# eudald-seeslab/mmsbm

Measured on AMD Instinct MI355X. Metric: EM iterations/sec (1M ratings, K=L=20), higher is better.
Workload: dtype f64; 1 GPU; C3: 1000000 synthetic ratings, 99997 users x 20000 items, R=5, K=20, L=20, one restart per GPU (sampling=1), uniform generator seed 0, model seed 0; launch=eager, pairs=99993, pair_stage=vector ALUs (pair_block_kernel)

## Files before the change

### mmsbm_amd/csrc/context.hpp

```cpp
#pragma once

namespace {

#define DISPATCH_GV(code, CALL)                                   \
  switch (code) {                                                 \
    case 0: CALL(4, 4); break;                                    \
    case 1: CALL(8, 4); break;                                    \
    case 2: CALL(16, 4); break;                                   \
    case 3: CALL(32, 4); break;                                   \
    case 4: CALL(64, 4); break;                                   \
    case 5: CALL(64, 8); break;                                   \
    default: CALL(64, 16); break;                                 \
  }

}

namespace mmsbm_hip_impl {

template <class T>
struct DevBuf {
  T *ptr = nullptr;
  size_t count = 0;
  DevBuf() = default;
  DevBuf(const DevBuf &) = delete;
// ... 153 lines not shown
}

inline void sort_unique_groups(std::vector<int32_t> &off, std::vector<int32_t> &val) {
  int32_t w = 0;
  for (size_t g = 0; g + 1 < off.size(); ++g) {
    const int32_t a = off[g], b = off[g + 1];
    std::sort(val.begin() + a, val.begin() + b);
    off[g] = w;
    for (int32_t e = a; e < b; ++e)
      if (e == a || val[e] != val[e - 1]) val[w++] = val[e];
  }
  off.back() = w;
  val.resize(static_cast<size_t>(w));
}

enum TimedCall { T_RECOMMEND = 0, T_FOLD_IN, T_POSITIONS, T_TOP_PAIRS, T_AUDIENCE, T_SIMILAR, T_OVERLAP, T_HELDOUT, T_EXPLAIN, T_DIVERSE, T_COUNT };

enum KernelId { K_SEG = 0, K_DENSE, K_ETAP, K_MATVEC_A, K_FUSED_PAIRS, K_FUSED_TAIL, K_COUNT };
const char *const kKernelNames[K_COUNT] = {"seg_pass_kernel", "pair_block_kernel(T+S)", "eta_p_kernel",
                                           "pair_block_kernel(A)", "pairs_fused_kernel", "tail_fused_kernel"};


}


struct mmsbm_hip_ctx {
  int device = 0;
  hipStream_t stream = nullptr;
  hipStream_t copy_stream = nullptr;
  hipStream_t xfer = nullptr;
  bool swapped = false;
  int64_t n_obs = 0;
  int ext_users = 0, ext_items = 0, ext_k = 0, ext_l = 0;
  int n_users = 0, n_items = 0, n_ratings = 0, k = 0, l = 0, kp = 0, lp = 0;
  int n_pairs = 0, n_chunks = 0;
  int code_k = 0, code_l = 0;
#ifdef MMSBM_ABLATE
  int ablate = 0;
#endif
  PairPlan pp;
  DevBuf<int32_t> grid_item;
  DevBuf<mmsbm::Chunk> grid_chunks;
  int grid_n_chunks = 0;
  DevBuf<double> btab;
  bool predict_fast = true;
  int seg_batch = 4;
  bool fused = false;
  bool fused_forced = false;
  bool fs_pairs = false, fs_users = false;
  DevBuf<mmsbm::FusedUnit> fp_units, fu_units;
  DevBuf<mmsbm::WorkItem> fp_items, fu_items;
  DevBuf<mmsbm::FusedSplit> fp_splits, fu_splits;
  int fp_max_parts = 0, fu_max_parts = 0, fu_blocks = 0;
  std::vector<char> a_ok;
  int nt_out = 7;
  int ranges_pairs = 1, ranges_users = 1;
  int n_cus = 256;
  bool gpu_layout = false;
  mmsbm::Layout lay;
  DevBuf<int32_t> pair_off, pair_user, pair_item, user_off, user_pair, item_off, item_pairs,
      item_deg, mv_chunk_off, orig_u, orig_i, orig_r;
  DevBuf<int32_t> item_grid;
  DevBuf<mmsbm::Chunk> mv_chunks;
  DevBuf<mmsbm::Chunk> lik_units;
  DevBuf<mmsbm::Chunk> a_chunks;
  int n_a_chunks = 0, a_units = 0;
  int n_lik_units = 0;
  DevBuf<mmsbm::WorkItem> pair_items, user_items;
  DevBuf<mmsbm::SplitSeg> pair_splits, user_splits;
  int n_slots = 1, sel = 0;
  int base_slot = 0, launch_slots = 1;
  SlotBuf pair_parts, user_parts;
  SlotBuf theta[2], eta[2], p[2], pt[2], atab[2], ctab, ttab, partial, npr;
  DevBuf<double> lik_part;
  DevBuf<double> lg_theta, lg_eta, lg_p;
  int lik_mode = 2;
  int lik_g = 0;
  PinBuf pin;
  std::unique_ptr<mmsbm_hip_impl::PredictSession> ps;
  std::unique_ptr<mmsbm_hip_impl::RecSession> rc;
  std::unique_ptr<mmsbm_hip_impl::SimSession> sm;
  std::unique_ptr<mmsbm_hip_impl::OvlSession> ov;
  std::unique_ptr<mmsbm_hip_impl::HoldSession> ho;
  std::unique_ptr<mmsbm_hip_impl::ExpSession> ex;
  float last_ms[T_COUNT] = {};
  int top_groups = 0;
  int64_t aud_rows = 0;
  int64_t aud_entries = 0;
  int64_t exp_rows = 0;
  int64_t div_rows = 0;
  DevBuf<double> snap_theta;
  SlotBuf snap_eta, snap_p;
  std::vector<char> snap_have;
  int cur = 0;
  std::vector<char> have;
  bool graph_mode = false;
  hipGraphExec_t graph_exec[2] = {nullptr, nullptr};
  bool profiling = false;
  std::vector<std::pair<int, std::pair<hipEvent_t, hipEvent_t>>> prof_events;

  void drop_graphs() {
    for (auto &g : graph_exec) {
      if (g) (void)hipGraphExecDestroy(g);
      g = nullptr;
    }
  }
// ... 65 lines not shown
```

### mmsbm_amd/csrc/launch.hpp

```cpp
#pragma once

namespace mmsbm_hip_impl {

void stage_seg(mmsbm_hip_ctx *c, bool commit, bool with_pairs, bool with_users, hipStream_t st);
void stage_dense_valu(mmsbm_hip_ctx *c);
void stage_dense_mfma(mmsbm_hip_ctx *c);
void stage_matvec_a_valu(mmsbm_hip_ctx *c, int slot, int a_slot, bool grid);
void stage_matvec_a_mfma(mmsbm_hip_ctx *c, int slot, int a_slot, bool grid);
int mfma_a_blocks_per_cu(const mmsbm_hip_ctx *c);
void stage_eta_p(mmsbm_hip_ctx *c, bool commit);
void stage_fused_pairs(mmsbm_hip_ctx *c);
void stage_fused_tail(mmsbm_hip_ctx *c, bool commit);
int likelihood_enqueue(mmsbm_hip_ctx *c);
void init_rows_launch(mmsbm_hip_ctx *c, const uint64_t pcg64_state[4]);
void omegas_launch(mmsbm_hip_ctx *c, double *dev_out, int64_t n_elems);
void prod_dist_launch(mmsbm_hip_ctx *c, const int32_t *du, const int32_t *di, double *dout, int64_t n_pairs);
int rows_launch(mmsbm_hip_ctx *c, int mode, const int32_t *pu, const int32_t *pi, const int32_t *preal,
                const double *weights, double *dist, double *block_out, int64_t n_rows, int first);
int score_rows_launch(mmsbm_hip_ctx *c, bool finish);
int score_stats_count();

void require_free_mem(size_t bytes, const std::string &what);
void recommend_begin(mmsbm_hip_ctx *c, const double *weights, int exclude_train);
void recommend_add(mmsbm_hip_ctx *c);
void recommend_query(mmsbm_hip_ctx *c, int64_t n_users, const int32_t *users, int n, int32_t *items, double *scores,
                     int32_t *counts);
void recommend_query_theta(mmsbm_hip_ctx *c, int64_t n_users, const double *theta, const int64_t *seen_offsets,
                           const int32_t *seen_items, int n, int32_t *items, double *scores, int32_t *counts);
void recommend_positions(mmsbm_hip_ctx *c, int64_t n_users, const int32_t *users, const int64_t *offsets,
                         const int32_t *items, int32_t *positions, int32_t *candidates);
void recommend_add_items(mmsbm_hip_ctx *c, int32_t n_new, const double *eta, const int64_t *seen_offsets,
                         const int32_t *seen_users);
void recommend_top_pairs(mmsbm_hip_ctx *c, int64_t n_users, const int32_t *users, int m, int32_t *out_users,
                         int32_t *out_items, double *out_scores, int32_t *count);
void recommend_query_items(mmsbm_hip_ctx *c, int64_t n_items, const int32_t *items, int n, int32_t *users,
                           double *scores, int32_t *counts);
void recommend_audience(mmsbm_hip_ctx *c, int64_t n_items, const int32_t *items, double min_score, int64_t capacity,
                        int64_t *offsets, int32_t *users, double *scores);
void recommend_query_within(mmsbm_hip_ctx *c, int64_t n_users, const int32_t *users, const int32_t *cand, int n_cand,
                            const int64_t *excl_offsets, const int32_t *excl_items, int n, int32_t *items,
                            double *scores, int32_t *counts);
void recommend_query_theta_within(mmsbm_hip_ctx *c, int64_t n_users, const double *theta, const int64_t *seen_offsets,
                                  const int32_t *seen_items, const int32_t *cand, int n_cand, int n, int32_t *items,
                                  double *scores, int32_t *counts);
void recommend_rank(mmsbm_hip_ctx *c, int64_t n_users, const int32_t *users, const int64_t *offsets,
                    const int32_t *cand, int n, int32_t *items, double *scores, int32_t *counts);
void similar_begin(mmsbm_hip_ctx *c, int side);
void similar_add(mmsbm_hip_ctx *c);
void similar_query(mmsbm_hip_ctx *c, int64_t n_rows, const int32_t *ids, int n, int32_t *out_ids, double *distance,
                   int32_t *counts);
void similar_pairs(mmsbm_hip_ctx *c, int64_t n_pairs, const int32_t *a, const int32_t *b, double *distance);
void recommend_diverse(mmsbm_hip_ctx *c, int64_t n_users, const int32_t *users, const int32_t *cand, int n_cand,
                       const int64_t *excl_offsets, const int32_t *excl_items, int n, int pool, double trade_off,
                       int32_t *items, double *scores, double *distances, int32_t *counts);
void overlap_begin(mmsbm_hip_ctx *c, int side);
void overlap_add(mmsbm_hip_ctx *c);
void overlap_query(mmsbm_hip_ctx *c, double *out);

void fold_in(mmsbm_hip_ctx *c, bool items_side, int64_t n_rows, const int32_t *user, const int32_t *item,
             const int32_t *rating, int32_t n_new, int32_t n_iters, double tol, const double *x0, double *x,
             int32_t *iters);

void heldout_begin(mmsbm_hip_ctx *c, int64_t n_rows, const int32_t *user, const int32_t *item, const int32_t *rating);
void heldout_eval(mmsbm_hip_ctx *c, int first, int n_slots, bool add, double *loglik);
void heldout_mean(mmsbm_hip_ctx *c, double *mean_p, double *loglik);
// ... 101 lines not shown
```

### mmsbm_amd/csrc/mmsbm_hip.hip

```cpp

#include "prelude.hpp"
#include "layout_gpu.hpp"
#include "pcg64.hpp"

#include <unistd.h>

#include <map>
#include <mutex>

namespace {

thread_local std::string g_last_error;

template <class F>
int guarded(F &&f) {
  try {
    f();
    return MMSBM_OK;
  } catch (const ApiError &e) {
    g_last_error = e.what();
    return e.code;
  } catch (const std::invalid_argument &e) {
    g_last_error = e.what();
    return MMSBM_E_INVALID;
// ... 81 lines not shown
}

}

namespace {

inline int balanced_run_units(const std::vector<int32_t> &rating_off, int slots, int lo, int hi) {
  int best = hi;
  double best_cost = 1e300;
  const bool align = mmsbm::chunk_align_on();
  const int n_ratings = static_cast<int>(rating_off.size()) - 1;
  for (int u = hi; u >= lo; --u) {
    long long wgs = 0;
    for (int r = 0; r < n_ratings; ++r)
      wgs += mmsbm::padded_chunk_count(rating_off[static_cast<size_t>(r) + 1] - rating_off[static_cast<size_t>(r)],
                                       u * kUnitPairs, n_ratings, align);
    const double cost = static_cast<double>((wgs + slots - 1) / std::max(slots, 1)) * (u + 0.6);
    if (cost < best_cost * 0.97) { best_cost = cost; best = u; }
  }
  return best;
}

void build_a_runs(mmsbm_hip_ctx *c, int units) {
  c->n_a_chunks = 0;
  c->a_chunks.release();
  if (!c->pp.mfma || c->n_pairs <= 0) return;
  const int now = c->pp.chunk_pairs / kUnitPairs, most = kMfmaChunkPairs / kUnitPairs;
  int a_units = units > 0 ? std::min(units, most)
                          : balanced_run_units(c->lay.rating_off, mfma_a_blocks_per_cu(c) * c->n_cus, std::max(2, now / 2),
                                               std::min(2 * now, most));
  c->a_units = a_units;
  if (a_units == now) return;
  mmsbm::Layout tmp;
  tmp.n_ratings = c->lay.n_ratings; tmp.rating_off = c->lay.rating_off;
  mmsbm::build_mv_chunks(tmp, a_units * kUnitPairs);
  c->a_chunks.upload(tmp.mv_chunks, c->stream);
  HIP_CHECK(hipStreamSynchronize(c->stream));
  c->n_a_chunks = static_cast<int>(tmp.mv_chunks.size());
}

bool fused_shape_ok(const mmsbm_hip_ctx *c) {
  return c->code_k <= 1 && c->code_l <= 1 && c->n_chunks > 0 && c->pp.fused_shape_ok();
}
bool fused_possible(const mmsbm_hip_ctx *c) {
  return fused_shape_ok(c) && (c->lay.pair_work.splits.empty() || c->fs_pairs) &&
         (c->lay.user_work.splits.empty() || c->fs_users);
}

void mark_a(mmsbm_hip_ctx *c, bool ok) {
  for (int s = c->base_slot; s < c->base_slot + c->launch_slots; ++s) c->a_ok[static_cast<size_t>(s)] = ok ? 1 : 0;
}

constexpr long long kFusedWorkMax = 14000000, kFusedWorkMaxSplit = 18000000, kFusedRatingsMax = 1500000;
bool use_fused(const mmsbm_hip_ctx *c) {
  const bool cut = !c->lay.pair_work.splits.empty() || !c->lay.user_work.splits.empty();
  return c->fused && fused_possible(c) &&
         (c->fused_forced || c->n_obs * c->launch_slots * (c->kp + c->lp) <= (cut ? kFusedWorkMaxSplit : kFusedWorkMax));
}

void launch_iteration(mmsbm_hip_ctx *c, bool commit) {
  if (use_fused(c)) {
    stage_fused_pairs(c);
    stage_fused_tail(c, commit);
    if (commit) c->cur ^= 1;
    mark_a(c, !commit);
    return;
  }
  ensure_a(c);
  stage_seg(c, commit, true, true, c->stream);
  stage_dense(c);
  stage_eta_p(c, commit);
  if (commit) {
    stage_matvec_a(c, c->cur ^ 1, c->cur ^ 1);
    c->cur ^= 1;
    mark_a(c, true);
  }
}

void run_iterations(mmsbm_hip_ctx *c, int n) {
  if (c->graph_mode && !c->profiling) {
    while (n >= 2) {
      const int slot = c->cur;
      if (!c->graph_exec[slot]) {
        if (!use_fused(c)) ensure_a(c);
        hipGraph_t graph = nullptr;
        HIP_CHECK(hipStreamBeginCapture(c->stream, hipStreamCaptureModeThreadLocal));
        try {
          launch_iteration(c, true);
          launch_iteration(c, true);
        } catch (...) {
          (void)hipStreamEndCapture(c->stream, &graph);
          if (graph) (void)hipGraphDestroy(graph);
          c->cur = slot;
          throw;
        }
        HIP_CHECK(hipStreamEndCapture(c->stream, &graph));
        hipError_t e = hipGraphInstantiate(&c->graph_exec[slot], graph, nullptr, nullptr, 0);
        (void)hipGraphDestroy(graph);
        if (e != hipSuccess)
          throw ApiError(MMSBM_E_HIP, std::string("hipGraphInstantiate: ") + hipGetErrorString(e));
      }
      HIP_CHECK(hipGraphLaunch(c->graph_exec[slot], c->stream));
      mark_a(c, !use_fused(c));
      n -= 2;
    }
  }
  for (; n > 0; --n) launch_iteration(c, true);
}

void require_params(const mmsbm_hip_ctx *c) {
  if (!c) throw std::invalid_argument("null context");
  if (!c->have[c->sel]) throw std::invalid_argument("set_params has not been called");
}
void require_all_params(const mmsbm_hip_ctx *c) {
  if (!c) throw std::invalid_argument("null context");
  for (int s = 0; s < c->n_slots; ++s)
    if (!c->have[s])
      throw std::invalid_argument(c->n_slots == 1 ? std::string("set_params has not been called")
                                                  : "set_params has not been called for slot " +
                                                        std::to_string(s));
}

void alloc_state(mmsbm_hip_ctx *c, int slots) {
// ... 434 lines not shown
                                            std::to_string(MMSBM_HIP_RECOMMEND_MAX_N) + " " + noun + " a query returns at most");
}

struct Option {
  const char *name;
  double (*get)(const mmsbm_hip_ctx *);
  void (*set)(mmsbm_hip_ctx *, double);
};
using Ctx = mmsbm_hip_ctx;
void set_audience(int64_t &field, const char *name, double v) {
  if (v < 0 || v > 2147483647.0 || v != std::floor(v)) throw std::invalid_argument(std::string(name) + ": 0 .. 2^31 - 1");
  field = static_cast<int64_t>(v);
}
const Option kOptions[] = {
    {"graph", [](const Ctx *c) -> double { return c->graph_mode; }, [](Ctx *c, double v) { c->graph_mode = v != 0.0; }},
    {"quad", [](const Ctx *c) -> double { return c->pp.quad_a; }, [](Ctx *c, double v) { c->pp.set_quad(v != 0.0); }},
    {"mfma", [](const Ctx *c) -> double { return c->pp.mfma ? 1.0 : (c->pp.mfma_big ? 2.0 : 0.0); },
     [](Ctx *c, double v) { c->pp.set_mfma(v); }},
    {"predict_fast", [](const Ctx *c) -> double { return c->predict_fast; }, [](Ctx *c, double v) { c->predict_fast = v != 0.0; }},
    {"fused", [](const Ctx *c) -> double { return c->fused; },
     [](Ctx *c, double v) {
       if (v != 0.0 && !fused_possible(c)) throw std::invalid_argument("fused: not available for this shape / data");
       c->fused = c->fused_forced = v != 0.0;
     }},
    {"nt_out", [](const Ctx *c) -> double { return nt_on(c); },
     [](Ctx *c, double v) {
       if (v < 0 || v > 15) throw std::invalid_argument("nt_out: 0 .. 15");
       c->nt_out = static_cast<int>(v);
     }},
    {"recommend_ms", [](const Ctx *c) -> double { return c->last_ms[T_RECOMMEND]; }, nullptr},
    {"fold_in_ms", [](const Ctx *c) -> double { return c->last_ms[T_FOLD_IN]; }, nullptr},
    {"position_ms", [](const Ctx *c) -> double { return c->last_ms[T_POSITIONS]; }, nullptr},
    {"similar_ms", [](const Ctx *c) -> double { return c->last_ms[T_SIMILAR]; }, nullptr},
    {"top_pairs_ms", [](const Ctx *c) -> double { return c->last_ms[T_TOP_PAIRS]; }, nullptr},
    {"overlap_ms", [](const Ctx *c) -> double { return c->last_ms[T_OVERLAP]; }, nullptr},
    {"heldout_ms", [](const Ctx *c) -> double { return c->last_ms[T_HELDOUT]; }, nullptr},
    {"audience_ms", [](const Ctx *c) -> double { return c->last_ms[T_AUDIENCE]; }, nullptr},
    {"explain_ms", [](const Ctx *c) -> double { return c->last_ms[T_EXPLAIN]; }, nullptr},
    {"diverse_ms", [](const Ctx *c) -> double { return c->last_ms[T_DIVERSE]; }, nullptr},
    {"top_pairs_groups", [](const Ctx *c) -> double { return c->top_groups; },
     [](Ctx *c, double v) {
       if (v < 0 || v > 4096 || v != std::floor(v)) throw std::invalid_argument("top_pairs_groups: 0 .. 4096");
       c->top_groups = static_cast<int>(v);
     }},
    {"audience_rows", [](const Ctx *c) -> double { return static_cast<double>(c->aud_rows); },
     [](Ctx *c, double v) { set_audience(c->aud_rows, "audience_rows", v); }},
    {"audience_entries", [](const Ctx *c) -> double { return static_cast<double>(c->aud_entries); },
     [](Ctx *c, double v) { set_audience(c->aud_entries, "audience_entries", v); }},
    {"explain_rows", [](const Ctx *c) -> double { return static_cast<double>(c->exp_rows); },
     [](Ctx *c, double v) { set_audience(c->exp_rows, "explain_rows", v); }},
    {"diverse_rows", [](const Ctx *c) -> double { return static_cast<double>(c->div_rows); },
     [](Ctx *c, double v) { set_audience(c->div_rows, "diverse_rows", v); }},
    {"launches", [](const Ctx *c) -> double { return use_fused(c) ? 2 : 4; }, nullptr},
    {"wide", [](const Ctx *c) -> double { return c->pp.wide; }, nullptr},
    {"lik_fast", [](const Ctx *c) -> double { return c->lik_mode; },
     [](Ctx *c, double v) {
       if (v != 0.0 && v != 1.0 && v != 2.0) throw std::invalid_argument("lik_fast: 0, 1 or 2");
       c->lik_mode = static_cast<int>(v);
     }},
    {"lik_g", [](const Ctx *c) -> double { return c->lik_g; },
     [](Ctx *c, double v) {
       const int g = static_cast<int>(v);
       if (g != 0 && g != 1 && g != 2 && g != 4 && g != 8) throw std::invalid_argument("lik_g: 0, 1, 2, 4 or 8");
       c->lik_g = g;
     }},
    {"ranges_pairs", [](const Ctx *c) -> double { return c->ranges_pairs; }, nullptr},
    {"ranges_users", [](const Ctx *c) -> double { return c->ranges_users; }, nullptr},
    {"chunk_pairs", [](const Ctx *c) -> double { return c->pp.chunk_pairs; }, nullptr},
    {"n_chunks", [](const Ctx *c) -> double { return c->n_chunks; }, nullptr},
    {"a_units", [](const Ctx *c) -> double { return c->a_units; },
     [](Ctx *c, double v) {
       if (v < 0 || v > kMfmaChunkPairs / kUnitPairs) throw std::invalid_argument("a_units: 0 .. 16");
       use_device(c);
       HIP_CHECK(hipStreamSynchronize(c->stream));
       build_a_runs(c, static_cast<int>(v));
     }},
    {"a_chunks", [](const Ctx *c) -> double { return c->n_a_chunks; }, nullptr},
    {"items_pairs", [](const Ctx *c) -> double { return static_cast<double>(c->lay.pair_work.items.size()); }, nullptr},
    {"items_users", [](const Ctx *c) -> double { return static_cast<double>(c->lay.user_work.items.size()); }, nullptr},
    {"splits_pairs", [](const Ctx *c) -> double { return static_cast<double>(c->lay.pair_work.splits.size()); }, nullptr},
    {"splits_users", [](const Ctx *c) -> double { return static_cast<double>(c->lay.user_work.splits.size()); }, nullptr},
    {"fused_split", [](const Ctx *c) -> double { return (c->fs_pairs ? 1 : 0) + (c->fs_users ? 2 : 0); }, nullptr},
    {"item_grid", [](const Ctx *c) -> double { return c->item_grid.count ? 1 : 0; }, nullptr},
    {"gpu_layout", [](const Ctx *c) -> double { return c->gpu_layout ? 1 : 0; }, nullptr},
};
const Option *find_option(const std::string &name) {
  for (const Option &o : kOptions)
    if (name == o.name) return &o;
  return nullptr;
}
void set_option(mmsbm_hip_ctx *ctx, const std::string &name, double value) {
  const Option *o = find_option(name);
  if (!o || !o->set) throw std::invalid_argument("unknown option: " + name);
  o->set(ctx, value);
  ctx->drop_graphs();
}
}


extern "C" {

int mmsbm_hip_abi_version(void) { return MMSBM_HIP_ABI_VERSION; }

#ifndef MMSBM_BUILD_ID
#define MMSBM_BUILD_ID "unknown"
#endif
// ... 1057 lines not shown
                            const int32_t *rating, int32_t n_new, int32_t n_iters, double tol,
                            const double *eta0, double *eta, int32_t *iters) {
  return fold_entry(ctx, true, n_rows, user, item, rating, n_new, n_iters, tol, eta0, eta, iters);
}

int mmsbm_hip_time_iterations(mmsbm_hip_ctx *ctx, int n_iters, float *elapsed_ms) {
  return guarded([&] {
    require_all_params(ctx);
    if (!elapsed_ms || n_iters < 0) throw std::invalid_argument("bad argument");
    use_device(ctx);
    EventPair ev;
    ev.start(ctx->stream);
    run_iterations(ctx, n_iters);
    ev.stop(ctx->stream);
    ev.wait();
    *elapsed_ms = ev.ms();
  });
}

int mmsbm_hip_kernel_count(void) { return K_COUNT; }

const char *mmsbm_hip_kernel_name(int index) {
  return (index >= 0 && index < K_COUNT) ? kKernelNames[index] : "";
}

int mmsbm_hip_profile_iterations(mmsbm_hip_ctx *ctx, int n_iters, float *mean_us,
                                 int *launches_per_iter) {
  return guarded([&] {
    require_all_params(ctx);
    if (!mean_us || n_iters <= 0) throw std::invalid_argument("bad argument");
    use_device(ctx);
    HIP_CHECK(hipStreamSynchronize(ctx->stream));
    ctx->profiling = true;
    try {
      for (int it = 0; it < n_iters; ++it) launch_iteration(ctx, true);
      HIP_CHECK(hipStreamSynchronize(ctx->stream));
    } catch (...) {
      ctx->profiling = false;
      throw;
    }
    ctx->profiling = false;
    collect_profile(ctx, mean_us, launches_per_iter, n_iters);
  });
}

int mmsbm_hip_kernel_bytes(const mmsbm_hip_ctx *ctx, int index, int64_t *bytes_read,
                           int64_t *bytes_written) {
  return guarded([&] {
    if (!ctx || !bytes_read || !bytes_written) throw std::invalid_argument("null argument");
    const int64_t N = ctx->n_obs, U = ctx->n_users, I = ctx->n_items, R = ctx->n_ratings;
    const int64_t K = ctx->k, L = ctx->l, Q = ctx->n_pairs;
    const int64_t C = static_cast<int64_t>(ctx->lay.mv_chunks.size());
    int64_t rd = 0, wr = 0;
    switch (index) {
      case K_SEG:
        rd = 2 * N * (4 + 8 * K) + (U + Q) * (8 * K + 4);
        wr = (U + Q) * 8 * K;
        break;
      case K_DENSE:
        rd = Q * (8 * K + 8 * L + 4) + C * 8 * K * L;
        wr = Q * 8 * L + C * 8 * K * L;
        break;
      case K_ETAP:
        rd = C * 8 * K * L + R * 8 * K * L + Q * (8 * L + 4) + I * (8 * L + 8);
        wr = 3 * R * 8 * K * L + I * 8 * L;
        break;
      case K_MATVEC_A: rd = Q * (8 * L + 4) + C * 8 * K * L; wr = Q * 8 * K; break;
      case K_FUSED_PAIRS:
        rd = Q * (8 * L + 4 + 4) + N * (4 + 8 * K) + 2 * C * 8 * K * L;
        wr = Q * (8 * K + 8 * L) + C * 8 * K * L;
        break;
      case K_FUSED_TAIL:
        rd = N * (4 + 8 * K) + U * (8 * K + 4) + C * 8 * K * L + R * 8 * K * L + Q * (8 * L + 4) + I * (8 * L + 8);
        wr = U * 8 * K + 3 * R * 8 * K * L + I * 8 * L;
        break;
      default: throw std::invalid_argument("kernel index out of range");
    }
    *bytes_read = rd * ctx->n_slots;
    *bytes_written = wr * ctx->n_slots;
  });
}

int mmsbm_hip_time_stage(mmsbm_hip_ctx *ctx, int stage, int reps, float *mean_us) {
  return guarded([&] {
    require_all_params(ctx);
#ifdef MMSBM_ABLATE
    ctx->ablate = stage >> 8;
    stage &= 0xff;
    struct Reset { mmsbm_hip_ctx *c; ~Reset() { c->ablate = 0; } } reset{ctx};
#else
    if (stage >> 8)
      throw ApiError(MMSBM_E_UNSUPPORTED, "time_stage: phase ablation (stage bits 8+) needs the diagnostic build (-DMMSBM_ABLATE, csrc/unity.hip)");
#endif
    if (!mean_us || reps <= 0 || stage < 0 || stage >= K_COUNT)
      throw std::invalid_argument("bad argument");
    if ((stage == K_FUSED_PAIRS || stage == K_FUSED_TAIL) && !fused_possible(ctx))
      throw std::invalid_argument("time_stage: the two-launch kernels do not apply to this shape / data");
    use_device(ctx);
    ensure_a(ctx);
    auto one = [&] {
      switch (stage) {
        case K_SEG: stage_seg(ctx, true, true, true, ctx->stream); break;
        case K_DENSE: stage_dense(ctx); break;
        case K_ETAP: stage_eta_p(ctx, true); break;
        case K_FUSED_PAIRS: stage_fused_pairs(ctx); break;
        case K_FUSED_TAIL: stage_fused_tail(ctx, true); break;
        default: stage_matvec_a(ctx, ctx->cur, ctx->cur ^ 1); break;
      }
    };
    for (int w = 0; w < 3; ++w) one();
    EventPair ev;
    ev.start(ctx->stream);
    for (int r = 0; r < reps; ++r) one();
    ev.stop(ctx->stream);
    ev.wait();
    *mean_us = ev.ms() * 1000.f / reps;
  });
}

int mmsbm_hip_set_option(mmsbm_hip_ctx *ctx, const char *name, double value) {
  return guarded([&] {
    if (!ctx || !name) throw std::invalid_argument("null argument");
    set_option(ctx, name, value);
  });
}

int mmsbm_hip_get_option(const mmsbm_hip_ctx *ctx, const char *name, double *value) {
  return guarded([&] {
    if (!ctx || !name || !value) throw std::invalid_argument("null argument");
    const Option *o = find_option(name);
    if (!o) throw std::invalid_argument(std::string("unknown option: ") + name);
    *value = o->get(ctx);
  });
}

int mmsbm_hip_set_graph_mode(mmsbm_hip_ctx *ctx, int enabled) {
  return guarded([&] {
    if (!ctx) throw std::invalid_argument("null context");
    set_option(ctx, "graph", enabled != 0);
  });
}

#ifdef MMSBM_STAMPS
int mmsbm_hip_debug_stamps(unsigned long long *out, int n_words) {
  return guarded([&] {
    HIP_CHECK(hipDeviceSynchronize());
    HIP_CHECK(hipMemcpyFromSymbol(out, HIP_SYMBOL(g_stamps), sizeof(unsigned long long) * n_words));
  });
}
#endif

struct mmsbm_hip_layout {
  mmsbm::Layout lay;
};

// ... 113 lines not shown
```

### mmsbm_amd/csrc/pair_plan.hpp

```cpp
#pragma once

namespace mmsbm_hip_impl {

#define MMSBM_PAIR_BLOCK_T_LIST(X)                                                                                     \
  X(1, false, 256, 2, false) X(1, false, 512, 2, false)                                                                \
  X(1, false, 256, 4, true) X(1, false, 512, 4, true) X(1, true, 256, 4, true) X(1, true, 512, 4, true)                \
  X(2, false, 256, 4, true) X(2, false, 512, 4, true) X(2, true, 256, 4, true) X(2, true, 512, 4, true)                \
  X(4, false, 512, 4, true)
#define MMSBM_PAIR_BLOCK_A_LIST(X)                                                                                     \
  X(1, false, 256, 4, false) X(1, false, 512, 4, false)                                                                \
  X(1, false, 256, 4, true) X(1, false, 512, 4, true) X(1, true, 256, 4, true) X(1, true, 512, 4, true)

constexpr int pair_block_key(int nacc, bool tlds, int nt, int kt, bool direct) {
  return nacc | (kt << 4) | (tlds ? 1 << 8 : 0) | (direct ? 1 << 9 : 0) | (nt << 10);
}
#define MMSBM_PB_LISTED(N, TL, NT, KT, D) case pair_block_key(N, TL, NT, KT, D):
inline bool pair_block_t_listed(int key) {
  switch (key) { MMSBM_PAIR_BLOCK_T_LIST(MMSBM_PB_LISTED) return true; default: return false; }
}
inline bool pair_block_a_listed(int key) {
  switch (key) { MMSBM_PAIR_BLOCK_A_LIST(MMSBM_PB_LISTED) return true; default: return false; }
}
#undef MMSBM_PB_LISTED

enum class PairForm { Wide, Block, Quad, Mfma, MfmaBig };

struct PairPlan {
  int kp = 0, lp = 0;
  int threads_t = kBlock, threads_a = kBlock;
  int kt = 4;
  int spb = kBlock, nacc = 1, nsub = 1;
  bool tl_t = false, tl_a = false;
  size_t lds_t = 0, lds_a = 0;
  bool direct_out = false;
  bool wide = false;
  bool mfma = false;
  bool mfma_big = false;
  bool quad_a = false;
  size_t lds_mt = 0, lds_ma = 0, lds_qa = 0;
  int chunk_pairs = mmsbm::kMvChunkPairs;

  bool big_tile() const { return tile_beyond_scalar_cache(kp, lp); }
  bool mfma_possible() const {
    return !wide && kp <= kMfmaMaxDim && lp <= kMfmaMaxDim && lds_mt <= kLdsMax && lds_ma <= kLdsMax;
  }
  bool quad_possible() const {
    return !wide && big_tile() && tl_a && threads_a == kPairBlockMax && lds_qa <= kLdsMax - 2048 && lp <= kQuadMaxL;
  }
  bool on_mfma() const { return mfma || mfma_big; }
  bool fused_shape_ok() const {
    return threads_t == kBlock && threads_a == kBlock && !tl_t && !tl_a && nacc == 1 && kt == 2 && spb * nsub <= kBlock &&
           !wide && !mfma && !mfma_big && !direct_out && chunk_pairs == mmsbm::kMvChunkPairs &&
           pairs_fused_lds(kp, lp) <= kLdsBudget;
  }

  PairForm form_t() const {
    return mfma_big ? PairForm::MfmaBig : mfma ? PairForm::Mfma : wide ? PairForm::Wide : PairForm::Block;
  }
  PairForm form_a() const { return (!on_mfma() && !wide && quad_a) ? PairForm::Quad : form_t(); }
  int key_t() const { return pair_block_key(nacc, tl_t, threads_t, kt, direct_out); }
  int key_a() const { return pair_block_key(1, tl_a, threads_a, 4, direct_out); }
  int quad_nl() const {
    const int nl = (lp + 3) / 4;
    return nl <= 8 ? 8 : nl <= 10 ? 10 : nl <= 12 ? 12 : nl <= 13 ? 13 : 14;
  }

  void set_mfma(double value) {
    mfma = value == 1.0 && mfma_possible();
    mfma_big = value != 0.0 && !mfma && chunk_pairs <= kMfmaChunkPairs;
  }
  void set_quad(bool on) { quad_a = on && quad_possible(); }
};

inline PairPlan plan_pair_shape(int kp, int lp, bool force_wide) {
  PairPlan p;
  p.kp = kp; p.lp = lp;
  auto threads_for = [](int nch) { return nch <= 6 ? kBlock : kPairBlockMax; };
  p.threads_t = threads_for(lp / 4);
  p.threads_a = threads_for(kp / 4);
  const int nthr = p.threads_t;
  p.kt = ((kp / 2) * (lp / 4) <= kBlock / 2) ? 2 : 4;
  const int nslot = (kp / p.kt) * (lp / 4);
  if (nslot <= nthr / 2) {
    p.spb = nslot; p.nacc = 1;
    const int room = (kp * (kUnitPairs + 1) + kUnitPairs * lp) / (nslot * 4 * p.kt);
    p.nsub = std::max(1, std::min(std::min(nthr / nslot, 8), 1 + room));
  } else {
    p.spb = nthr;
    int n = 1;
    while (n * nthr < nslot) n *= 2;
    p.nacc = n;
  }
  p.tl_t = tile_in_lds(kp, lp);
  p.tl_a = tile_in_lds(lp, kp);
  p.lds_t = pair_block_lds(kp, lp, p.tl_t);
  p.lds_a = pair_block_lds(lp, kp, p.tl_a);
  if (p.lds_t > kLdsMax) { p.tl_t = false; p.lds_t = pair_block_lds(kp, lp, false); }
  if (p.lds_a > kLdsMax) { p.tl_a = false; p.lds_a = pair_block_lds(lp, kp, false); }
  p.wide = p.lds_t > kLdsMax || p.lds_a > kLdsMax || p.nacc > 4 || force_wide;
  return p;
}

inline PairPlan plan_pair_forms(PairPlan p, int n_pairs, int n_cus, bool no_mfma, int mfma_chunk) {
  const bool big_tile = p.big_tile();
  p.lds_mt = pair_mfma_lds(p.kp, p.lp, true);
  p.lds_ma = pair_mfma_lds(p.lp, p.kp, false);
// ... 14 lines not shown
```

### mmsbm_amd/csrc/tu_fused.hip

```cpp
#include "prelude.hpp"
#include "seg_pass.hpp"
#include "pair_block.hpp"
#include "eta_p.hpp"
#include "fused_small.hpp"

namespace mmsbm_hip_impl {

void stage_fused_pairs(mmsbm_hip_ctx *c) {
  LaunchScope ls(c, K_FUSED_PAIRS, true);
  const int s = c->base_slot, cur = c->cur;
  FusedPairArgs fa{};
  fa.pt_tiles = c->pt[cur].at(s); fa.p_tiles = c->p[cur].at(s); fa.eta = c->eta[cur].at(s);
  fa.theta = theta_tab(c, cur); fa.a_out = a_tab(c, cur);
  fa.pair_off = c->pair_off.ptr; fa.pair_user = c->pair_user.ptr; fa.pair_item = c->pair_item.ptr;
  fa.chunks = c->mv_chunks.ptr; fa.t_out = c->ttab.at(s); fa.partial = c->partial.at(s);
  fa.kp = c->kp; fa.lp = c->lp; fa.spb = c->pp.spb; fa.nsub = c->pp.nsub; fa.nt = nt_on(c) & 1;
  fa.bs_tiles = c->p[0].stride; fa.bs_eta = c->eta[0].stride; fa.bs_t = c->ttab.stride; fa.bs_partial = c->partial.stride;
  const bool split = c->fs_pairs && !c->lay.pair_work.splits.empty();
  fa.units = split ? c->fp_units.ptr : nullptr; fa.items = split ? c->fp_items.ptr : nullptr;
  fa.splits = split ? c->fp_splits.ptr : nullptr;
  const size_t lds = pairs_fused_lds(c->kp, c->lp, split ? c->fp_max_parts : 0);
  const dim3 grid = slot_grid(c, c->n_chunks);
#define PF(G, S)                                                                  \
  do {                                                                            \
    allow_big_lds(pairs_fused_kernel<G, 4, S>, lds);                              \
    LAUNCH_IN(ls, (pairs_fused_kernel<G, 4, S>), grid, kBlock, lds, c->stream, fa); \
  } while (0)
  if (c->code_k == 0) { if (split) PF(4, true); else PF(4, false); }
  else { if (split) PF(8, true); else PF(8, false); }
#undef PF
  ls.done();
}
void stage_fused_tail(mmsbm_hip_ctx *c, bool commit) {
  LaunchScope ls(c, K_FUSED_TAIL, true);
  const SegArgs su = seg_users_args(c, commit, c->n_users);
  const EtaPArgs a = eta_p_args(c, commit, kRedCols);
  const int per_u = kBlock / group_lanes(c->code_k), per_i = kBlock / group_lanes(c->code_l);
  const bool split = c->fs_users && !c->lay.user_work.splits.empty();
  const int bu = split ? c->fu_blocks : (su.nseg + per_u - 1) / per_u, nb_i = (c->n_items + per_i - 1) / per_i;
  const dim3 grid = slot_grid(c, bu + a.nb_p + nb_i);
  const FusedUserArgs fu{split ? c->fu_units.ptr : nullptr, split ? c->fu_items.ptr : nullptr, split ? c->fu_splits.ptr : nullptr};
  const size_t lds = split ? static_cast<size_t>(c->fu_max_parts) * c->kp * sizeof(double) : 0;
  const bool deep = static_cast<long long>(grid.x) * grid.y <= c->n_cus;
#define TAIL(G, V, GL, VL)                                                                                        \
  do {                                                                                                            \
    if (split) {                                                                                                  \
      allow_big_lds(tail_fused_kernel<G, V, GL, VL, 16, true>, lds);                                              \
      LAUNCH_IN(ls, (tail_fused_kernel<G, V, GL, VL, 16, true>), grid, kBlock, lds, c->stream, su, a, bu, c->kp, fu); \
    } else if (deep) LAUNCH_IN(ls, (tail_fused_kernel<G, V, GL, VL, 32, false>), grid, kBlock, 0, c->stream, su, a, bu, c->kp, fu); \
    else LAUNCH_IN(ls, (tail_fused_kernel<G, V, GL, VL, 16, false>), grid, kBlock, 0, c->stream, su, a, bu, c->kp, fu);      \
  } while (0)
  switch (c->code_k * 2 + c->code_l) {
    case 0: TAIL(4, 4, 4, 4); break;
    case 1: TAIL(4, 4, 8, 4); break;
    case 2: TAIL(8, 4, 4, 4); break;
    default: TAIL(8, 4, 8, 4); break;
  }
#undef TAIL
  ls.done();
}

}
```

Measured before the change: 10650 it/s.

## Merge pair segment pass and dense tile stage into one kernel for large shapes

Adds a pass_dense kernel that, per chunk of pairs, computes the pair-side theta gather and normalisation, builds the T output and the partial K×L tile sums in LDS, and runs the user segment pass as extra blocks of the same launch. It replaces the separate stage_seg and stage_dense launches on commit iterations when the shape qualifies (code_k==1, no splits, work at or above a threshold). The aim is to cut one launch and avoid writing and re-reading the pair-side intermediate through global memory. The cost is heavier LDS use and lower occupancy per block. The two-launch fused path and the original path are left as they were.

Result: faster. 11840 it/s, median of 6 (+11.2%).

```diff
diff --git a/mmsbm_amd/csrc/context.hpp b/mmsbm_amd/csrc/context.hpp
--- a/mmsbm_amd/csrc/context.hpp
+++ b/mmsbm_amd/csrc/context.hpp
@@ -229,6 +229,7 @@
   DevBuf<mmsbm::WorkItem> fp_items, fu_items;
   DevBuf<mmsbm::FusedSplit> fp_splits, fu_splits;
   int fp_max_parts = 0, fu_max_parts = 0, fu_blocks = 0;
+  int pass_dense = -1;
   std::vector<char> a_ok;
   int nt_out = 7;
   int ranges_pairs = 1, ranges_users = 1;
diff --git a/mmsbm_amd/csrc/launch.hpp b/mmsbm_amd/csrc/launch.hpp
--- a/mmsbm_amd/csrc/launch.hpp
+++ b/mmsbm_amd/csrc/launch.hpp
@@ -11,6 +11,7 @@
 void stage_eta_p(mmsbm_hip_ctx *c, bool commit);
 void stage_fused_pairs(mmsbm_hip_ctx *c);
 void stage_fused_tail(mmsbm_hip_ctx *c, bool commit);
+void stage_pass_dense(mmsbm_hip_ctx *c);
 int likelihood_enqueue(mmsbm_hip_ctx *c);
 void init_rows_launch(mmsbm_hip_ctx *c, const uint64_t pcg64_state[4]);
 void omegas_launch(mmsbm_hip_ctx *c, double *dev_out, int64_t n_elems);
diff --git a/mmsbm_amd/csrc/mmsbm_hip.hip b/mmsbm_amd/csrc/mmsbm_hip.hip
--- a/mmsbm_amd/csrc/mmsbm_hip.hip
+++ b/mmsbm_amd/csrc/mmsbm_hip.hip
@@ -157,10 +157,24 @@
 }
 
 constexpr long long kFusedWorkMax = 14000000, kFusedWorkMaxSplit = 18000000, kFusedRatingsMax = 1500000;
+
+bool pass_dense_possible(const mmsbm_hip_ctx *c) {
+  return c->launch_slots == 1 && c->code_k == 1 && c->code_l <= 1 && c->n_chunks > 0 && c->pp.pass_dense_shape_ok() &&
+         c->lay.pair_work.items.empty() && c->lay.user_work.items.empty() && c->lay.pair_work.splits.empty() &&
+         c->lay.user_work.splits.empty();
+}
+constexpr long long kPassDenseWorkMin = 20000000;
+static_assert(kPassDenseWorkMin > kFusedWorkMaxSplit, "no shape changes from two launches to three");
+
 bool use_fused(const mmsbm_hip_ctx *c) {
   const bool cut = !c->lay.pair_work.splits.empty() || !c->lay.user_work.splits.empty();
+  if (c->pass_dense == 1 && !c->fused_forced && pass_dense_possible(c)) return false;
   return c->fused && fused_possible(c) &&
          (c->fused_forced || c->n_obs * c->launch_slots * (c->kp + c->lp) <= (cut ? kFusedWorkMaxSplit : kFusedWorkMax));
+}
+bool use_pass_dense(const mmsbm_hip_ctx *c) {
+  if (c->pass_dense == 0 || use_fused(c) || !pass_dense_possible(c)) return false;
+  return c->pass_dense == 1 || c->n_obs * (c->kp + c->lp) >= kPassDenseWorkMin;
 }
 
 void launch_iteration(mmsbm_hip_ctx *c, bool commit) {
@@ -172,8 +186,12 @@
     return;
   }
   ensure_a(c);
-  stage_seg(c, commit, true, true, c->stream);
-  stage_dense(c);
+  if (commit && use_pass_dense(c)) {
+    stage_pass_dense(c);
+  } else {
+    stage_seg(c, commit, true, true, c->stream);
+    stage_dense(c);
+  }
   stage_eta_p(c, commit);
   if (commit) {
     stage_matvec_a(c, c->cur ^ 1, c->cur ^ 1);
@@ -714,6 +732,11 @@
     {"diverse_rows", [](const Ctx *c) -> double { return static_cast<double>(c->div_rows); },
      [](Ctx *c, double v) { set_audience(c->div_rows, "diverse_rows", v); }},
     {"launches", [](const Ctx *c) -> double { return use_fused(c) ? 2 : 4; }, nullptr},
+    {"pass_dense", [](const Ctx *c) -> double { return use_pass_dense(c) ? 1 : 0; },
+     [](Ctx *c, double v) {
+       if (v != -1.0 && v != 0.0 && v != 1.0) throw std::invalid_argument("pass_dense: -1, 0 or 1");
+       c->pass_dense = static_cast<int>(v);
+     }},
     {"wide", [](const Ctx *c) -> double { return c->pp.wide; }, nullptr},
     {"lik_fast", [](const Ctx *c) -> double { return c->lik_mode; },
      [](Ctx *c, double v) {
@@ -1877,12 +1900,18 @@
     const int64_t K = ctx->k, L = ctx->l, Q = ctx->n_pairs;
     const int64_t C = static_cast<int64_t>(ctx->lay.mv_chunks.size());
     int64_t rd = 0, wr = 0;
+    const bool merged = use_pass_dense(ctx);
     switch (index) {
       case K_SEG:
         rd = 2 * N * (4 + 8 * K) + (U + Q) * (8 * K + 4);
         wr = (U + Q) * 8 * K;
+        if (merged) {
+          rd += Q * (8 * L + 4) + C * 8 * K * L;
+          wr += Q * (8 * L - 8 * K) + C * 8 * K * L;
+        }
         break;
       case K_DENSE:
+        if (merged) break;
         rd = Q * (8 * K + 8 * L + 4) + C * 8 * K * L;
         wr = Q * 8 * L + C * 8 * K * L;
         break;
@@ -1923,9 +1952,17 @@
       throw std::invalid_argument("time_stage: the two-launch kernels do not apply to this shape / data");
     use_device(ctx);
     ensure_a(ctx);
+    const bool merged = use_pass_dense(ctx);
+    if (merged && stage == K_DENSE) {
+      *mean_us = 0.f;
+      return;
+    }
     auto one = [&] {
       switch (stage) {
-        case K_SEG: stage_seg(ctx, true, true, true, ctx->stream); break;
+        case K_SEG:
+          if (merged) stage_pass_dense(ctx);
+          else stage_seg(ctx, true, true, true, ctx->stream);
+          break;
         case K_DENSE: stage_dense(ctx); break;
         case K_ETAP: stage_eta_p(ctx, true); break;
         case K_FUSED_PAIRS: stage_fused_pairs(ctx); break;
diff --git a/mmsbm_amd/csrc/pair_plan.hpp b/mmsbm_amd/csrc/pair_plan.hpp
--- a/mmsbm_amd/csrc/pair_plan.hpp
+++ b/mmsbm_amd/csrc/pair_plan.hpp
@@ -52,6 +52,10 @@
     return threads_t == kBlock && threads_a == kBlock && !tl_t && !tl_a && nacc == 1 && kt == 2 && spb * nsub <= kBlock &&
            !wide && !mfma && !mfma_big && !direct_out && chunk_pairs == mmsbm::kMvChunkPairs &&
            pairs_fused_lds(kp, lp) <= kLdsBudget;
+  }
+  bool pass_dense_shape_ok() const {
+    return form_t() == PairForm::Block && threads_t == kBlock && !tl_t && nacc == 1 && kt == 2 && spb * nsub <= kBlock &&
+           !direct_out && chunk_pairs == mmsbm::kMvChunkPairs && kUnitPairs * lp <= 3 * 2 * kBlock && lds_t <= kLdsBudget;
   }
 
   PairForm form_t() const {
diff --git a/mmsbm_amd/csrc/pass_dense.hpp b/mmsbm_amd/csrc/pass_dense.hpp
--- /dev/null
+++ b/mmsbm_amd/csrc/pass_dense.hpp
@@ -0,0 +1,217 @@
+#pragma once
+
+namespace {
+
+struct PassDenseArgs {
+  RowTab a_fixed;
+  RowTab theta;
+  const int32_t *pair_off, *pair_user, *pair_item;
+  const mmsbm::Chunk *chunks;
+  const double *p_tiles;
+  const double *eta;
+  double *t_out;
+  double *partial;
+  int kp, lp, spb, nsub;
+  int nt;
+  int n_units;
+};
+
+template <int G, int VEC>
+__device__ __forceinline__ void pass_dense_unit(const PassDenseArgs &pa, int unit) {
+  constexpr int CS = kUnitPairs + 1, KT = 2, TV = KT * 4, B = 4;
+  constexpr int NGRP = kBlock / G, ROUNDS = kUnitPairs / NGRP;
+  constexpr int CH = (G < 16) ? 2 * G : G;
+  constexpr int NE = 3;
+  const int kp = pa.kp, lp = pa.lp;
+  extern __shared__ double lds[];
+  double *cst = lds;
+  double *es = cst + static_cast<size_t>(kp) * CS;
+  double *tout = es;
+  const mmsbm::Chunk ch = pa.chunks[unit];
+  const int tid = threadIdx.x, wave = tid >> 6, lane = tid & 63;
+  const int q0 = ch.q_begin, np = ch.q_end - ch.q_begin;
+  const int grp = tid / G, gl = tid % G;
+  typedef const double __attribute__((address_space(4))) * const_tile_ptr;
+  const const_tile_ptr gtile = (const_tile_ptr)(reinterpret_cast<uintptr_t>(
+      pa.p_tiles + static_cast<size_t>(ch.rating) * kp * lp));
+
+  int beg[ROUNDS], end[ROUNDS], ids[NE];
+  const int tot = np * lp;
+#pragma unroll
+  for (int r = 0; r < ROUNDS; ++r) {
+    const int p = grp + r * NGRP;
+    beg[r] = p < np ? pa.pair_off[q0 + p] : 0;
+    end[r] = p < np ? pa.pair_off[q0 + p + 1] : 0;
+  }
+#pragma unroll
+  for (int j = 0; j < NE; ++j) {
+    const int t = min(tid * 2 + j * kBlock * 2, max(tot - 2, 0));
+    ids[j] = tot > 0 ? pa.pair_item[q0 + t / lp] : 0;
+  }
+  const auto eta_row = [&](int j) {
+    const int t = min(tid * 2 + j * kBlock * 2, max(tot - 2, 0));
+    return *reinterpret_cast<const double2 *>(pa.eta + static_cast<size_t>(ids[j]) * lp + t % lp);
+  };
+  const double2 ev0 = eta_row(0), ev1 = eta_row(1), ev2 = eta_row(2);
+  int m0, m1;
+  {
+    const int cnt = min(CH, end[0] - beg[0]);
+    m0 = cnt > 0 ? pa.pair_user[beg[0] + min(gl, cnt - 1)] : 0;
+    m1 = (CH > G && cnt > 0) ? pa.pair_user[beg[0] + min(G + gl, cnt - 1)] : 0;
+  }
+  __builtin_amdgcn_sched_barrier(0);
+  if (tid * 2 < tot) *reinterpret_cast<double2 *>(es + tid * 2) = ev0;
+  if (tid * 2 + kBlock * 2 < tot) *reinterpret_cast<double2 *>(es + tid * 2 + kBlock * 2) = ev1;
+  if (tid * 2 + kBlock * 4 < tot) *reinterpret_cast<double2 *>(es + tid * 2 + kBlock * 4) = ev2;
+
+  const bool act = gl * VEC < kp;
+  const int lane_off = act ? gl * VEC : 0;
+  const bool g_main = lane_off < pa.theta.mw;
+  const double *gbase = g_main ? pa.theta.main + lane_off : pa.theta.tail + (lane_off - pa.theta.mw);
+  const size_t gstride = g_main ? pa.theta.rs_m : pa.theta.rs_t;
+#pragma unroll
+  for (int r = 0; r < ROUNDS; ++r) {
+    const int p = grp + r * NGRP;
+    double f[VEC], acc[VEC];
+#pragma unroll
+    for (int v = 0; v < VEC; ++v) acc[v] = 0.0;
+    if (p < np) {
+      load_vec_in<VEC>(rowtab_ptr(pa.a_fixed, static_cast<size_t>(q0 + p), lane_off), f, (pa.nt & 2) != 0);
+      if (!act) {
+#pragma unroll
+        for (int v = 0; v < VEC; ++v) f[v] = 0.0;
+      }
+      int mine0 = m0, mine1 = m1;
+      if (r > 0) {
+        const int cnt = min(CH, end[r] - beg[r]);
+        mine0 = cnt > 0 ? pa.pair_user[beg[r] + min(gl, cnt - 1)] : 0;
+        mine1 = (CH > G && cnt > 0) ? pa.pair_user[beg[r] + min(G + gl, cnt - 1)] : 0;
+      }
+      for (int c0 = beg[r]; c0 < end[r]; c0 += CH) {
+        const int cnt = min(CH, end[r] - c0);
+        for (int n = 0; n < cnt; n += B) {
+          double g[B][VEC];
+#pragma unroll
+          for (int b = 0; b < B; ++b) {
+            const int jj = min(n + b, cnt - 1);
+            const int id = __shfl((CH > G && jj >= G) ? mine1 : mine0, jj, G);
+            load_vec<VEC>(gbase + static_cast<size_t>(id) * gstride, g[b]);
+          }
+#pragma unroll
+          for (int b = 0; b < B; ++b) {
+            if (n + b < cnt) {
+              double pt = 0.0;
+#pragma unroll
+              for (int v = 0; v < VEC; ++v) pt = fma(g[b][v], f[v], pt);
+              const double s = group_sum<G>(pt);
+              const double w = 1.0 / fmax(s, kEps);
+#pragma unroll
+              for (int v = 0; v < VEC; ++v) acc[v] = fma(g[b][v], w, acc[v]);
+            }
+          }
+        }
+        if (c0 + CH < end[r]) {
+          const int c1 = c0 + CH, cn = min(CH, end[r] - c1);
+          mine0 = pa.pair_user[c1 + min(gl, cn - 1)];
+          mine1 = (CH > G) ? pa.pair_user[c1 + min(G + gl, cn - 1)] : 0;
+        }
+      }
+    }
+    if (act) {
+#pragma unroll
+      for (int v = 0; v < VEC; ++v) cst[(lane_off + v) * CS + p] = acc[v];
+    }
+  }
+  __syncthreads();
+
+  const int nch = lp >> 2;
+  const int nslot = (kp / KT) * nch, spb = pa.spb, nsub = pa.nsub;
+  const int sub = tid / spb, slot0 = tid % spb;
+  const bool s_active = sub < nsub;
+  const int o = min(slot0, nslot - 1);
+  const int coff = (o / nch) * KT * CS, eoff = (o % nch) * 4;
+  double sacc[TV];
+#pragma unroll
+  for (int j = 0; j < TV; ++j) sacc[j] = 0.0;
+  if (s_active) {
+#pragma unroll 2
+    for (int j = sub; j < np; j += nsub) {
+      double cv[KT];
+#pragma unroll
+      for (int i = 0; i < KT; ++i) cv[i] = cst[coff + i * CS + j];
+      const double2 e0 = *reinterpret_cast<const double2 *>(es + j * lp + eoff);
+      const double2 e1 = *reinterpret_cast<const double2 *>(es + j * lp + eoff + 2);
+#pragma unroll
+      for (int i = 0; i < KT; ++i) {
+        sacc[4 * i + 0] = fma(cv[i], e0.x, sacc[4 * i + 0]);
+        sacc[4 * i + 1] = fma(cv[i], e0.y, sacc[4 * i + 1]);
+        sacc[4 * i + 2] = fma(cv[i], e1.x, sacc[4 * i + 2]);
+        sacc[4 * i + 3] = fma(cv[i], e1.y, sacc[4 * i + 3]);
+      }
+    }
+  }
+  __syncthreads();
+  for (int c = __builtin_amdgcn_readfirstlane(wave); c < nch; c += kBlock / 64) {
+    double a0 = 0.0, a1 = 0.0, a2 = 0.0, a3 = 0.0;
+    for (int d = 0; d < kp; d += 4) {
+      double x[4];
+      double2 t0[4], t1[4];
+#pragma unroll
+      for (int i = 0; i < 4; ++i) {
+        x[i] = cst[(d + i) * CS + lane];
+        const const_tile_ptr row = gtile + static_cast<size_t>(d + i) * lp + c * 4;
+        t0[i].x = row[0]; t0[i].y = row[1];
+        t1[i].x = row[2]; t1[i].y = row[3];
+      }
+#pragma unroll
+      for (int i = 0; i < 4; ++i) {
+        a0 = fma(x[i], t0[i].x, a0);
+        a1 = fma(x[i], t0[i].y, a1);
+        a2 = fma(x[i], t1[i].x, a2);
+        a3 = fma(x[i], t1[i].y, a3);
+      }
+    }
+    double2 w0, w1;
+    w0.x = a0; w0.y = a1; w1.x = a2; w1.y = a3;
+    *reinterpret_cast<double2 *>(tout + lane * lp + c * 4) = w0;
+    *reinterpret_cast<double2 *>(tout + lane * lp + c * 4 + 2) = w1;
+  }
+  __syncthreads();
+  {
+    double *dst = pa.t_out + static_cast<size_t>(q0) * lp;
+    for (int t = tid * 2; t < tot; t += kBlock * 2)
+      store_out2(dst + t, *reinterpret_cast<const double2 *>(tout + t), (pa.nt & 1) != 0);
+  }
+  if (nsub > 1) {
+    __syncthreads();
+    if (s_active && sub > 0 && slot0 < nslot) {
+#pragma unroll
+      for (int j = 0; j < TV; ++j) lds[(j * (nsub - 1) + sub - 1) * nslot + slot0] = sacc[j];
+    }
+    __syncthreads();
+    if (sub == 0 && slot0 < nslot) {
+      for (int oo = 1; oo < nsub; ++oo)
+#pragma unroll
+        for (int j = 0; j < TV; ++j) sacc[j] += lds[(j * (nsub - 1) + oo - 1) * nslot + slot0];
+    }
+  }
+  if (sub == 0 && slot0 < nslot) {
+    double *cell = pa.partial + static_cast<size_t>(unit) * kp * lp + (o / nch) * KT * lp + eoff;
+#pragma unroll
+    for (int h = 0; h < KT; ++h) {
+      double2 x, y;
+      x.x = sacc[4 * h]; x.y = sacc[4 * h + 1]; y.x = sacc[4 * h + 2]; y.y = sacc[4 * h + 3];
+      *reinterpret_cast<double2 *>(cell + h * lp) = x;
+      *reinterpret_cast<double2 *>(cell + h * lp + 2) = y;
+    }
+  }
+}
+
+template <int G, int VEC>
+__global__ __launch_bounds__(kBlock, 6) void pass_dense_kernel(PassDenseArgs pa, SegArgs su, int dp) {
+  const int bx = static_cast<int>(blockIdx.x);
+  if (bx < pa.n_units) pass_dense_unit<G, VEC>(pa, bx);
+  else seg_body<G, VEC, 4, 1>(su, (bx - pa.n_units) * (kBlock / G) + threadIdx.x / G, dp, 1);
+}
+
+}
diff --git a/mmsbm_amd/csrc/tu_fused.hip b/mmsbm_amd/csrc/tu_fused.hip
--- a/mmsbm_amd/csrc/tu_fused.hip
+++ b/mmsbm_amd/csrc/tu_fused.hip
@@ -3,6 +3,7 @@
 #include "pair_block.hpp"
 #include "eta_p.hpp"
 #include "fused_small.hpp"
+#include "pass_dense.hpp"
 
 namespace mmsbm_hip_impl {
 
@@ -60,4 +61,24 @@
   ls.done();
 }
 
+void stage_pass_dense(mmsbm_hip_ctx *c) {
+  LaunchScope ls(c, K_SEG, true);
+  const int s = c->base_slot, cur = c->cur, nt = nt_on(c);
+  PassDenseArgs pa{};
+  pa.a_fixed = a_tab(c, cur); pa.theta = theta_tab(c, cur);
+  pa.pair_off = c->pair_off.ptr; pa.pair_user = c->pair_user.ptr; pa.pair_item = c->pair_item.ptr;
+  pa.chunks = c->mv_chunks.ptr; pa.p_tiles = c->p[cur].at(s); pa.eta = c->eta[cur].at(s);
+  pa.t_out = c->ttab.at(s); pa.partial = c->partial.at(s);
+  pa.kp = c->kp; pa.lp = c->lp; pa.spb = c->pp.spb; pa.nsub = c->pp.nsub;
+  pa.nt = (nt & 1) | ((nt & 4) ? 2 : 0);
+  const SegArgs su = seg_users_args(c, true, c->n_users);
+  const int per = kBlock / group_lanes(c->code_k);
+  pa.n_units = static_cast<int>(c->lay.mv_chunks.size());
+  const int bu = (su.nseg + per - 1) / per;
+  allow_big_lds(pass_dense_kernel<8, 4>, c->pp.lds_t);
+  LAUNCH_IN(ls, (pass_dense_kernel<8, 4>), dim3(static_cast<unsigned>(pa.n_units + bu), 1, 1), kBlock,
+            c->pp.lds_t, c->stream, pa, su, c->kp);
+  ls.done();
 }
+
+}
```
